# wq2012/SpectralCluster

Hardware: AMD Instinct MI355X
Metric: predict() calls/sec, n=8192 d=256 ICASSP2018 (GraphCut, eigengap k in [2,20], cosine k-means) (higher is better)
Workload: dtype f64; 1 GPU; icassp2018_graphcut_n8192_d256_k8_max20; n_samples=8192, n_features=256, parallelism=replicas x1, collectives=none

## Files before the change

### include/spectralcluster_amd.h

```cpp
#ifndef SPECTRALCLUSTER_AMD_H_
#define SPECTRALCLUSTER_AMD_H_

#include <stddef.h>
#include <stdint.h>

#ifdef __cplusplus
extern "C" {
#endif

#define SC_ABI_VERSION 10
#define SC_MAX_OPS 16
#define SC_MAX_BLUR_RADIUS 32
#define SC_MAX_EIG 128
#define SC_MAX_STAGES 16

typedef struct sc_handle_s* sc_handle;

typedef enum sc_status {
  SC_OK = 0,
  SC_ERR_INVALID = -1,
  SC_ERR_OOM = -2,
  SC_ERR_HIP = -3,
  SC_ERR_NOT_CONVERGED = -4,
  SC_ERR_UNSUPPORTED = -5,
// ... 368 lines not shown
  SC_FRONT_INFO_FREE_FORMS_S = 9,
  SC_FRONT_INFO_CROP_SOURCE = 10,
  SC_FRONT_INFO_CUT_KERNEL = 11,
  SC_FRONT_INFO_WRITTEN = 12,
  SC_FRONT_INFO_LAUNCHES = 13,
  SC_FRONT_INFO_COUNT = 16
};
typedef struct sc_front_out {
  double* a0;
  double* cropval;
  double* cut;
  double* a;
  double* s;
  double* rowmax;
  double* rowsum;
  double* c;
  double* p;
  double* t;
  int32_t info[SC_FRONT_INFO_COUNT];
} sc_front_out;
int sc_stage_front(sc_handle h, int route, const sc_config* cfg, int count, const int32_t* ns,
                   int d, const double* const* xs, const double* affinity,
                   const double* p_values, sc_front_out* outs);
enum { SC_TD_BACKTRANSFORM_GLOBAL = 1 };
int sc_stage_tridiag(sc_handle h, const double* m, int n, const double* c, const double* p,
                     double* d, double* e, double* tau, double* reflectors);
int sc_stage_tridiag_values(sc_handle h, const double* d, const double* e, int n,
                            double* values_desc);
int sc_stage_td_backtransform(sc_handle h, const double* reflectors, const double* tau, int n,
                              double* z, int cols, int flags);
int sc_stage_laplacian(sc_handle h, int laplacian_type, const double* in, int n,
                       double* out);
int sc_stage_sym_eig(sc_handle h, const double* m, int n, int count, int descend,
                     double* values, double* vectors, sc_diag* diag);
int sc_stage_eig(sc_handle h, const double* m, int n, int count, int descend,
                 double* values, double* vectors, sc_diag* diag);
int sc_random_state_doubles(uint32_t seed, int count, double* out);
int sc_uniform_choice(int n, double u);
int sc_host_symmetric_eig(const double* a, int m, double* values, double* vectors);
int sc_host_symmetric_eig_partial(const double* a, int m, int need, double* values,
                                  double* vectors);
int sc_host_tridiag_eigvectors(const double* d, const double* e, int n, const double* lam,
                               int k, double* vectors);
int sc_host_general_eig(const double* a, int m, int nvec, double* values_re, double* values_im,
                        double* vectors_re, double* vectors_im);
int sc_host_general_eig_fast(const double* a, int m, int nvec, double* values_re,
// ... 68 lines not shown
```

### spectralcluster_amd/_lib.py

```python

from __future__ import annotations

import ctypes
import os
import threading
import typing

import numpy as np

SC_MAX_OPS = 16
SC_MAX_BLUR_RADIUS = 32
SC_MAX_EIG = 128
SC_MAX_STAGES = 16

SC_OK = 0
SC_ERR_INVALID = -1
SC_ERR_OOM = -2
SC_ERR_HIP = -3
SC_ERR_NOT_CONVERGED = -4
SC_ERR_UNSUPPORTED = -5
SC_ERR_NON_FINITE = -6

STAGE_NAMES = ("affinity", "refine", "diffuse", "scaling", "eig", "kmeans",
               "total", "blur", "threshold_sym", "matvec", "affinity_gemm",
# ... 186 lines not shown
    "sc_last_error": (ctypes.c_char_p, [_handle_t]),
    "sc_synchronize": (ctypes.c_int, [_handle_t]),
    "sc_set_profiling": (ctypes.c_int, [_handle_t, ctypes.c_int]),
    "sc_set_diffuse_mode": (ctypes.c_int, [_handle_t, ctypes.c_int]),
    "sc_set_free_prune": (ctypes.c_int, [_handle_t, ctypes.c_int]),
    "sc_stage_diffuse_rowstats": (ctypes.c_int, [_handle_t, _c_double_p, ctypes.c_int,
                                                 ctypes.c_int, _c_double_p, _c_double_p,
                                                 ctypes.POINTER(ctypes.c_int32)]),
    "sc_stage_block_operator": (ctypes.c_int, [_handle_t, ctypes.c_int,
                                               ctypes.POINTER(ctypes.c_int32),
                                               ctypes.POINTER(_c_double_p),
                                               ctypes.POINTER(_c_double_p),
                                               ctypes.POINTER(_c_double_p),
                                               ctypes.POINTER(_c_double_p),
                                               ctypes.POINTER(_c_double_p),
                                               ctypes.POINTER(_c_double_p), ctypes.c_int]),
    "sc_stage_krylov_state": (ctypes.c_int, [_handle_t, ctypes.POINTER(ctypes.c_int32),
                                             _c_double_p, _c_double_p, _c_double_p, _c_double_p,
                                             _c_double_p]),
    "sc_stage_front": (ctypes.c_int, [_handle_t, ctypes.c_int, ctypes.POINTER(ScConfig),
                                      ctypes.c_int, ctypes.POINTER(ctypes.c_int32), ctypes.c_int,
                                      ctypes.POINTER(_c_double_p), _c_double_p, _c_double_p,
                                      ctypes.POINTER(ScFrontOut)]),
    "sc_stage_tridiag": (ctypes.c_int, [_handle_t, _c_double_p, ctypes.c_int, _c_double_p,
                                        _c_double_p, _c_double_p, _c_double_p, _c_double_p,
                                        _c_double_p]),
    "sc_stage_tridiag_values": (ctypes.c_int, [_handle_t, _c_double_p, _c_double_p, ctypes.c_int,
                                               _c_double_p]),
    "sc_stage_td_backtransform": (ctypes.c_int, [_handle_t, _c_double_p, _c_double_p,
                                                 ctypes.c_int, _c_double_p, ctypes.c_int,
                                                 ctypes.c_int]),
    "sc_config_default": (ctypes.c_int, [ctypes.POINTER(ScConfig)]),
    "sc_gaussian_weights": (ctypes.c_int, [ctypes.c_double,
                                           ctypes.POINTER(ctypes.c_int32),
                                           _c_double_p]),
    "sc_predict": (ctypes.c_int, [_handle_t, _c_double_p, ctypes.c_int, ctypes.c_int,
                                  ctypes.POINTER(ScConfig), _c_int64_p,
                                  ctypes.POINTER(ScDiag)]),
    "sc_set_embeddings": (ctypes.c_int, [_handle_t, _c_double_p, ctypes.c_int,
                                         ctypes.c_int]),
    "sc_predict_array": (ctypes.c_int, [_handle_t, ctypes.POINTER(ScArray),
                                        ctypes.POINTER(ScConfig), _c_int64_p,
                                        ctypes.POINTER(ScDiag)]),
    "sc_set_embeddings_array": (ctypes.c_int, [_handle_t, ctypes.POINTER(ScArray)]),
    "sc_predict_batch_arrays": (ctypes.c_int, [_handle_t, ctypes.POINTER(ScArray), ctypes.c_int,
                                               ctypes.POINTER(ScConfig),
# ... 496 lines not shown
```

### spectralcluster_amd/csrc/api.hip

```cpp
#include <algorithm>
#include <array>
#include <cmath>
#include <cstdio>
#include <cstdlib>
#include <cstring>
#include <vector>

#include <condition_variable>
#include <mutex>
#include <string>
#include <thread>

#include "handle.h"
#include "host_pool.h"

int ensure_matrices(sc_handle h, int n, int d, bool affinity_copy) {
  h->krylov_m = 0;
  const size_t ldn = matrix_ld(n);
  const size_t nn = (size_t)n * ldn * sizeof(double);
  if (affinity_copy) SC_TRY(grow(h, h->A0, nn));
  SC_TRY(grow(h, h->B1, nn));
  SC_TRY(grow(h, h->B2, nn));
  if (d > 0) {
    const size_t ldx = round_up(d, 16);
// ... 591 lines not shown
  hipStream_t s = h->stream;
  const double* cur = ptr<double>(h->A0);
  double* bufs[2] = {ptr<double>(h->B1), ptr<double>(h->B2)};
  int which = 0;
  bool symmetric = h->affinity_symmetric;
  const bool constrain_after = constraint_active(h, cfg, false);
  bool folded_rownorm = false;
  int e_begin, e_after_refine;
  const bool fine = h->profile_level >= 2;
  int eb0 = -1, eb1 = -1, et0 = -1, et1 = -1;
  h->n_mv_ev = 0;
  bool free_path = false;
  const double* amax_of = nullptr;
  const double* digits_of = nullptr;
  float diffuse_ms_events[SC_MAX_OPS][2];
  int n_diffuse = 0;
  ev_rec(h, &e_begin);
  const bool blur_fast = (cfg->blur_radius == 4 || cfg->blur_radius == 8) && n >= 128;
  const double* pending_diag = nullptr;
  bool have_partials = false;
  bool have_row_stats = false;
  int crop_source = 0, cut_kernel = 0;
  h->last_blur = BlurLaunch();
  if (resume) {
    cur = resume->matrix;
    symmetric = resume->symmetric;
    folded_rownorm = resume->folded_rownorm;
    which = resume->scratch == bufs[0] ? 0 : 1;
    if (resume->free_op) h->free_checked = false;
  }
  for (int i = 0; i < (resume ? 0 : cfg->n_ops); ++i) {
    const int op = cfg->ops[i];
    const int next = i + 1 < cfg->n_ops ? cfg->ops[i + 1] : 0;
    const int next2 = i + 2 < cfg->n_ops ? cfg->ops[i + 2] : 0;
    const bool thr_sym_fusable = true;
    const bool partials_usable = cfg->threshold_type == SC_THRESHOLD_ROW_MAX &&
                                 !cfg->preserve_diagonal;
    if (op == SC_OP_ROW_WISE_NORMALIZE && symmetric && i == cfg->n_ops - 1 &&
        !constrain_after) {
      folded_rownorm = true;
      continue;
    }
    if (op == SC_OP_CROP_DIAGONAL && next == SC_OP_GAUSSIAN_BLUR && blur_fast) {
      if (cur == ptr<double>(h->A0) && h->have_cropval) {
        pending_diag = ptr<double>(h->cropval);
        crop_source = 1;
      } else {
        launch_crop_value(s, cur, n, ld, ptr<double>(h->dvec));
        pending_diag = ptr<double>(h->dvec);
        crop_source = 2;
      }
      have_partials = false;
      continue;
    }
    double* out = bufs[which];
    which ^= 1;
    int e0 = -1, e1 = -1;
    bool keep_cur = false;
    if (op == SC_OP_DIFFUSE) ev_rec(h, &e0);
    if (op == SC_OP_GAUSSIAN_BLUR && blur_fast) {
      const bool want = next == SC_OP_ROW_WISE_THRESHOLD && next2 == SC_OP_SYMMETRIZE &&
                        partials_usable;
      SC_TRY(upload_blur_weights(h, cfg));
      if (fine) ev_rec(h, &eb0);
      have_partials = launch_gaussian_blur_fused(s, cur, out, n, ld, cfg->blur_radius,
                                                 ptr<double>(h->blurw), pending_diag,
                                                 want ? ptr<double>(h->rmpart) : nullptr,
                                                 &h->last_blur);
      if (fine) ev_rec(h, &eb1);
      pending_diag = nullptr;
      SC_TRY(check_last(h, "blur launch"));
    } else if (op == SC_OP_ROW_WISE_THRESHOLD && next == SC_OP_SYMMETRIZE && thr_sym_fusable) {
      if (cfg->threshold_type == SC_THRESHOLD_PERCENTILE)
        launch_cut_percentile(s, cur, n, ld, cfg->p_percentile, ptr<double>(h->cut),
                              cfg->preserve_diagonal);
      else if (have_partials && partials_usable)
        launch_cut_from_partials(s, ptr<double>(h->rmpart), n,
                                 blur_tile_columns(n, cfg->blur_radius),
                                 cfg->p_percentile, ptr<double>(h->cut));
      else
        launch_cut_from_rows(s, cur, n, ld, cfg->p_percentile, ptr<double>(h->cut),
                             cfg->preserve_diagonal);
      cut_kernel = cfg->threshold_type == SC_THRESHOLD_PERCENTILE
                       ? 3 : (have_partials && partials_usable ? 1 : 2);
      const bool amax_known =
          cfg->threshold_type == SC_THRESHOLD_ROW_MAX && h->affinity_from_embeddings &&
          !h->constraint_applied && cfg->p_percentile > 0.0 && cfg->soft_multiplier >= 0.0 &&
          cfg->soft_multiplier <= 1.0 && i + 2 < cfg->n_ops && cfg->ops[i + 2] == SC_OP_DIFFUSE &&
          free_diffuse_wanted(h, cfg, n, make_eig_request(cfg));
      const bool fuse_digits =
          amax_known && !constrain_after && !front_only &&
          (i + 2 == cfg->n_ops - 1 ||
           (i + 2 == cfg->n_ops - 2 && cfg->ops[i + 3] == SC_OP_ROW_WISE_NORMALIZE));
      const double amax_floor = (cfg->binarize || cfg->preserve_diagonal) ? 1.0 : 0.0;
      if (fuse_digits)
        SC_TRY(free_fused_prepare(h, s, n, ptr<double>(h->cut), cfg->p_percentile, amax_floor));
      if (fine) ev_rec(h, &et0);
      if (fuse_digits)
        launch_threshold_symmetrize_digits(s, cur, out, n, ld, ptr<double>(h->cut),
                                           cfg->soft_multiplier, cfg->binarize,
                                           cfg->symmetrize_type, cfg->preserve_diagonal,
                                           ptr<signed char>(h->fq), ptr<double>(h->fscal),
                                           ptr<double>(h->fypart), ptr<int>(h->frpart),
                                           ptr<double>(h->fq2part), ptr<double>(h->fmx64));
      else
        launch_threshold_symmetrize(s, cur, out, n, ld, ptr<double>(h->cut),
                                    cfg->soft_multiplier, cfg->binarize, cfg->symmetrize_type,
                                    cfg->preserve_diagonal);
      if (fine) ev_rec(h, &et1);
      SC_TRY(check_last(h, "threshold+symmetrize launch"));
      if (fuse_digits) {
        amax_of = out;
        digits_of = out;
      } else if (amax_known) {
        SC_TRY(ensure_free(h, n));
        launch_free_amax_from_cut(s, ptr<double>(h->cut), n, cfg->p_percentile, amax_floor,
                                  ptr<double>(h->fscal));
        amax_of = out;
      }
      have_partials = false;
      cur = out;
// ... 641 lines not shown
```

### spectralcluster_amd/csrc/blur.hip

```cpp
#include <algorithm>
#include <cstring>

#include "dpp.h"
#include "sc_internal.h"

namespace sc {

constexpr int TH = 32;
constexpr int TW = 64;


__global__ __launch_bounds__(256) void k_gaussian_blur(
    const double* __restrict__ in, double* __restrict__ out, int n, int ld,
    int radius, const double* __restrict__ weights) {
  extern __shared__ __attribute__((aligned(16))) double smem[];
  const int R = radius;
  const int HW = TW + 2 * R;
  const int HH = TH + 2 * R;
  double* tile = smem;
  double* mid = smem + HH * HW;
  double* w = mid + TH * HW;

  const int i0 = blockIdx.y * TH;
  const int j0 = blockIdx.x * TW;
// ... 130 lines not shown
#pragma unroll
      for (int e = 0; e < 4; ++e) dst[e] = row[gjin[e]];
    }
    if (diag != nullptr) {
#pragma unroll
      for (int e = 0; e < 4; ++e)
        if (gjin[e] == gi) dst[e] = diag[gi];
    }
  };
  double win[S][4];
#pragma unroll
  for (int q = 0; q < S - 1; ++q) load_row(r0 - R + q, win[q]);
  const int gjo0 = j0 + q0 - R;
  const bool lane_ok = q0 >= R && q0 + 3 < 256 - R;
  const bool full_store = lane_ok && gjo0 + 3 < n;
  for (int o = r0; o < rend; o += S) {
#pragma unroll
    for (int u = 0; u < S; ++u) {
      const int gi = o + u;
      if (gi >= rend) break;
      load_row(gi + R + kAhead, win[(u + S - 1) % S]);
      double t[4];
#pragma unroll
      for (int e = 0; e < 4; ++e) {
        double acc = win[(u + R) % S][e] * w[0];
#pragma unroll
        for (int j = R; j >= 1; --j)
          acc += (win[(u + R - j) % S][e] + win[(u + R + j) % S][e]) * w[j];
        t[e] = acc;
      }
      double ext[(2 * NB + 1) * 4];
#pragma unroll
      for (int e = 0; e < 4; ++e) ext[NB * 4 + e] = t[e];
#pragma unroll
      for (int e = 0; e < 4; ++e) {
        double below = t[e], above = t[e];
#pragma unroll
        for (int d = 1; d <= NB; ++d) {
          below = lane_from_below(below);
          above = lane_from_above(above);
          ext[(NB - d) * 4 + e] = below;
          ext[(NB + d) * 4 + e] = above;
        }
      }
      double res[4];
      double m = -INFINITY;
#pragma unroll
      for (int e = 0; e < 4; ++e) {
        double acc = ext[NB * 4 + e] * w[0];
#pragma unroll
        for (int j = R; j >= 1; --j)
          acc += (ext[NB * 4 + e - j] + ext[NB * 4 + e + j]) * w[j];
        res[e] = acc;
        if (lane_ok && gjo0 + e < n) m = fmax(m, acc);
      }
      double* orow = out + (size_t)gi * ld + gjo0;
      if (out == nullptr) {
      } else if (full_store) {
        *reinterpret_cast<double2*>(orow) = make_double2(res[0], res[1]);
        *reinterpret_cast<double2*>(orow + 2) = make_double2(res[2], res[3]);
      } else if (lane_ok) {
#pragma unroll
        for (int e = 0; e < 4; ++e)
          if (gjo0 + e < n) orow[e] = res[e];
      }
      if (rowmax != nullptr) {
        m = wave_max_to_last(m);
        if (lane == 63) rowmax[(size_t)gi * ncols + bx] = m;
      }
    }
  }
}
template <int R>
__global__ __launch_bounds__(256) void k_gaussian_blur_stream(
    const double* __restrict__ in, double* __restrict__ out, int n, int ld,
// ... 37 lines not shown
  if (j >= n) return;
  auto at = [&](int e) { return AXIS == 0 ? in[(size_t)e * ld + j] : in[(size_t)i * ld + e]; };
  out[(size_t)i * ld + j] = blur_line_point(at, AXIS == 0 ? i : j, n, radius, weights);
}

void launch_gaussian_blur_any_radius(hipStream_t s, const double* in, double* tmp, double* out,
                                     int n, int ld, int radius, const double* weights_dev) {
  dim3 grid((n + 255) / 256, n);
  hipLaunchKernelGGL(k_gaussian_blur_axis<0>, grid, dim3(256), 0, s, in, tmp, n, ld, radius,
                     weights_dev);
  hipLaunchKernelGGL(k_gaussian_blur_axis<1>, grid, dim3(256), 0, s, tmp, out, n, ld, radius,
                     weights_dev);
}

void launch_gaussian_blur(hipStream_t s, const double* in, double* out, int n,
                          int ld, int radius, const double* weights_dev) {
  launch_gaussian_blur_fused(s, in, out, n, ld, radius, weights_dev, nullptr, nullptr);
}

int blur_tile_columns(int n, int radius) {
  const int ow = (n >= kStreamMinN ? 256 : 64) - 2 * radius;
  return (n + ow - 1) / ow;
}

bool launch_gaussian_blur_fused(hipStream_t s, const double* in, double* out, int n, int ld,
                                int radius, const double* weights_dev, const double* diag,
                                double* rowmax_partials, BlurLaunch* taken) {
  dim3 grid((n + TW - 1) / TW, (n + TH - 1) / TH);
  if (taken) *taken = BlurLaunch{0, 0};
  if ((radius == 4 || radius == 8) && n >= kStreamMinN) {
    const int strips = blur_tile_columns(n, radius);
    int rows = stream_rows_per_wave((long long)strips * n, radius);
    const int per_round = 256 * (radius == 4 ? 3 : 2);
    while (rows < kStreamRowsMax) {
      const long long wgs = (long long)strips * ((n + 4 * rows - 1) / (4 * rows));
      if (wgs <= per_round || wgs % per_round == 0 || wgs % per_round > per_round * 3 / 4) break;
      ++rows;
    }
    dim3 sgrid(strips, (n + 4 * rows - 1) / (4 * rows));
    if (taken) *taken = BlurLaunch{2, rows};
    if (radius == 4)
      hipLaunchKernelGGL((k_gaussian_blur_stream<4>), sgrid, dim3(256), 0, s, in, out, n, ld,
                         weights_dev, diag, rowmax_partials, rows);
    else
      hipLaunchKernelGGL((k_gaussian_blur_stream<8>), sgrid, dim3(256), 0, s, in, out, n, ld,
                         weights_dev, diag, rowmax_partials, rows);
// ... 63 lines not shown
```

### spectralcluster_amd/csrc/handle.h

```cpp
#ifndef SPECTRALCLUSTER_AMD_HANDLE_H_
#define SPECTRALCLUSTER_AMD_HANDLE_H_

#include <algorithm>
#include <array>
#include <cmath>
#include <cstdio>
#include <cstdlib>
#include <cstring>
#include <string>
#include <vector>

#include "sc_internal.h"

using namespace sc;

struct DevBuf {
  void* p = nullptr;
  size_t bytes = 0;
};

constexpr int kKgenBufs = 12;
constexpr int kGroupBanks = 2;
constexpr int kGroupLanes = 3;

// ... 93 lines not shown
  int gconv_hist[16] = {0};
  int gconv_seen = 0;
  hipEvent_t ev[48];
  int nev = 0;
  StageEvents stage_events;
  int profile_level = 1;
  int mv_ev[16][2];
  int n_mv_ev = 0;
  int aff_ev[2] = {-1, -1};
  int blurw_radius = -1;
  double blurw_host[2 * SC_MAX_BLUR_RADIUS + 1];
  int krnd_k = -1, krnd_trials = -1;
  int kfirst_n = -1, kfirst = 0;
  int diffuse_mode = -1;
  DevBuf fq, ft32, fy1, fR, fscal, fwords, fcand, fY, fsplit, fypart, frpart;
  int free_prune = -1;
  DevBuf fq2part, fmx64, ftau64, fplan;
  int* h_free = nullptr;
  bool free_checked = false;
  int free_ev[5] = {-1, -1, -1, -1, -1};
  int krylov_m = 0, krylov_n = 0, krylov_cycles = 0, krylov_ahead = 0;
  bool krylov_free = false;
  BlurLaunch last_blur;
};

inline void ev_rec(sc_handle h, int* slot) {
  if (h->nev < 48) {
    hipEventRecord(h->ev[h->nev], h->stream);
    *slot = h->nev++;
  } else {
    *slot = -1;
  }
}
inline float ev_ms(sc_handle h, int a, int b) {
  if (a < 0 || b < 0) return 0.f;
  float ms = 0.f;
  hipEventElapsedTime(&ms, h->ev[a], h->ev[b]);
  return ms;
}

constexpr int kTilemapTableMax = 64;
constexpr int kMaxCols = 128;
inline int matrix_ld(int n) {
  int ld = round_up(n, 16);
  if (ld % 512 == 0) ld += 16;
  return ld;
// ... 245 lines not shown
```

### spectralcluster_amd/csrc/rowops.hip

```cpp
#include <algorithm>
#include <cstring>

#include "dpp.h"
#include "sc_internal.h"

namespace sc {

constexpr int kRowThreads = 256;

__device__ __forceinline__ double wave_max(double v) {
#pragma unroll
  for (int o = 32; o > 0; o >>= 1) v = fmax(v, __shfl_xor(v, o));
  return v;
}
__device__ __forceinline__ double wave_sum(double v) {
#pragma unroll
  for (int o = 32; o > 0; o >>= 1) v += __shfl_xor(v, o);
  return v;
}
__device__ __forceinline__ double block_max(double v, double* sm) {
  v = wave_max(v);
  __syncthreads();
  if ((threadIdx.x & 63) == 0) sm[threadIdx.x >> 6] = v;
  __syncthreads();
// ... 313 lines not shown
    hb[w] = (signed char)h;
    lb[w] = (signed char)l;
  }
  signed char* dst = dg.Q + (size_t)row * dg.pitch + (size_t)blk * 128 + c0;
  *reinterpret_cast<short*>(dst) = (short)((unsigned char)hb[0] | ((unsigned short)(unsigned char)hb[1] << 8));
  *reinterpret_cast<short*>(dst + 64) = (short)((unsigned char)lb[0] | ((unsigned short)(unsigned char)lb[1] << 8));
  const double ys = half_sum_to_last(v0 + v1);
  const int rs = half_sum_to_last(qv[0] + qv[1]);
  const double q2s = half_sum_to_last(q2);
  if (lane0) {
    dg.ypart[(size_t)blk * (kTsTile * dg.nblk) + row] = ys;
    dg.rpart[(size_t)blk * (kTsTile * dg.nblk) + row] = rs;
    dg.q2part[(size_t)blk * (kTsTile * dg.nblk) + row] = q2s;
  }
  return q2s;
}
__device__ __forceinline__ void ts_store_mx(const TsDigits& dg, const double* sm, int group,
                                            int blk) {
  double m = sm[0];
#pragma unroll
  for (int u = 1; u < 8; ++u) m = fmax(m, sm[u]);
  dg.mx64[(size_t)group * dg.nblk + blk] = sqrt(m) * (1.0 + 0x1p-52);
}
template <bool DIGITS>
__device__ __forceinline__ void threshold_symmetrize_body(
    const double* __restrict__ in, double* __restrict__ out, int n, int ld,
    const double* __restrict__ cut, double mult, int binarize, int symtype, int ntiles,
    int preserve_diag, const TsDigits dg) {
  __shared__ double tT[kTsTile][kTsTile + 1];
  __shared__ double smax[2][8];
  double q2m = 0.0;
  const bool digits = DIGITS && dg.Q != nullptr;
  const int id = blockIdx.x;
  const double b2 = 2.0 * ntiles + 1.0;
  int ti = (int)((b2 - sqrt(b2 * b2 - 8.0 * id)) * 0.5);
  ti = ti < 0 ? 0 : (ti >= ntiles ? ntiles - 1 : ti);
  auto off = [&](int t) { return t * ntiles - (t * (t - 1)) / 2; };
  while (ti > 0 && off(ti) > id) --ti;
  while (ti + 1 < ntiles && off(ti + 1) <= id) ++ti;
  const int tj = ti + (id - off(ti));
  const int bi = ti * kTsTile, bj = tj * kTsTile;
  const int tx = threadIdx.x & 31, ty = threadIdx.x >> 5;
  const int c0 = 2 * tx;
  const bool diag_tile = ti == tj;
  double2 a[8], b[8];
  double ca[8], cb[8];
#pragma unroll
  for (int q = 0; q < 8; ++q) {
    const int r = ty + 8 * q;
    const int gi = bi + r, gj = bj + c0;
    a[q] = (gi < n && gj < n) ? *reinterpret_cast<const double2*>(in + (size_t)gi * ld + gj)
                              : make_double2(0.0, 0.0);
    ca[q] = gi < n ? cut[gi] : 0.0;
  }
  if (!diag_tile) {
#pragma unroll
    for (int q = 0; q < 8; ++q) {
      const int r = ty + 8 * q;
      const int gi = bj + r, gj = bi + c0;
      b[q] = (gi < n && gj < n) ? *reinterpret_cast<const double2*>(in + (size_t)gi * ld + gj)
                                : make_double2(0.0, 0.0);
      cb[q] = gi < n ? cut[gi] : 0.0;
    }
  }
  auto thr = [&](double v, double c, int gi, int gj) {
    if (!(gi < n && gj < n)) return 0.0;
    v = v < c ? v * mult : (binarize ? 1.0 : v);
    if (preserve_diag && gi == gj) v = 1.0;
    return v;
  };
#pragma unroll
  for (int q = 0; q < 8; ++q) {
    const int r = ty + 8 * q;
    a[q].x = thr(a[q].x, ca[q], bi + r, bj + c0);
    a[q].y = thr(a[q].y, ca[q], bi + r, bj + c0 + 1);
    if (diag_tile) {
      b[q] = a[q];
    } else {
      b[q].x = thr(b[q].x, cb[q], bj + r, bi + c0);
      b[q].y = thr(b[q].y, cb[q], bj + r, bi + c0 + 1);
    }
    tT[r][c0] = b[q].x;
    tT[r][c0 + 1] = b[q].y;
  }
  __syncthreads();
  double sigma = 0.0;
  if (digits) {
// ... 27 lines not shown
#pragma unroll
  for (int q = 0; q < 8; ++q) {
    const int r = ty + 8 * q;
    tT[r][c0] = a[q].x;
    tT[r][c0 + 1] = a[q].y;
  }
  __syncthreads();
#pragma unroll
  for (int q = 0; q < 8; ++q) {
    const int r = ty + 8 * q;
    const int gi = bj + r, gj = bi + c0;
    const double2 o = make_double2(tT[c0][r], tT[c0 + 1][r]);
    if (gi < n && gj + 1 < n)
      *reinterpret_cast<double2*>(out + (size_t)gi * ld + gj) = o;
    else if (gi < n && gj < n)
      out[(size_t)gi * ld + gj] = o.x;
    if (digits) q2m = fmax(q2m, ts_digits(dg, sigma, gi, ti, c0, o.x, o.y, tx == 31));
  }
  if (digits) {
    if (tx == 31) smax[1][ty] = q2m;
    __syncthreads();
    if (threadIdx.x == 0) ts_store_mx(dg, smax[1], tj, ti);
  }
}
__global__ __launch_bounds__(256) void k_threshold_symmetrize(
    const double* __restrict__ in, double* __restrict__ out, int n, int ld,
    const double* __restrict__ cut, double mult, int binarize, int symtype, int ntiles,
    int preserve_diag) {
  threshold_symmetrize_body<false>(in, out, n, ld, cut, mult, binarize, symtype, ntiles,
                                   preserve_diag, TsDigits{});
}
__global__ __launch_bounds__(256) void k_threshold_symmetrize_digits(
    const double* __restrict__ in, double* __restrict__ out, int n, int ld,
    const double* __restrict__ cut, double mult, int binarize, int symtype, int ntiles,
    int preserve_diag, const TsDigits dg) {
  threshold_symmetrize_body<true>(in, out, n, ld, cut, mult, binarize, symtype, ntiles,
                                  preserve_diag, dg);
}
__device__ __forceinline__ void free_partials_reduce_body(
    const double* __restrict__ ypart, const int* __restrict__ rpart, int n, int nblk,
    double* __restrict__ y1, double* __restrict__ R, unsigned long long* __restrict__ rmax_bits,
    const FreeSegs segs) {
  __shared__ double sy[4][64];
  __shared__ double sq[4][64];
  __shared__ long long sr[4][64];
  const int r = threadIdx.x & 63, qd = threadIdx.x >> 6;
// ... 573 lines not shown
                     cut, mult, binarize, preserve_diag);
}
void launch_threshold_symmetrize(hipStream_t s, const double* in, double* out, int n, int ld,
                                 const double* cut, double mult, int binarize, int symtype,
                                 int preserve_diag) {
  const int t = (n + kTsTile - 1) / kTsTile;
  hipLaunchKernelGGL(k_threshold_symmetrize, dim3(t * (t + 1) / 2), dim3(256), 0, s, in, out,
                     n, ld, cut, mult, binarize, symtype, t, preserve_diag);
}
void launch_threshold_symmetrize_digits(hipStream_t s, const double* in, double* out, int n, int ld,
                                        const double* cut, double mult, int binarize, int symtype,
                                        int preserve_diag, signed char* Q, double* scal,
                                        double* ypart, int* rpart, double* q2part,
                                        double* mx64) {
  const int t = (n + kTsTile - 1) / kTsTile;
  const size_t pitch = (size_t)2 * t * kTsTile;
  const int rows_padded = (n + 127) / 128 * 128;
  if (rows_padded > t * kTsTile)
    hipMemsetAsync(Q + (size_t)t * kTsTile * pitch, 0, (size_t)(rows_padded - t * kTsTile) * pitch, s);
  const TsDigits dg{Q, pitch, t, scal, ypart, rpart, q2part, mx64};
  hipLaunchKernelGGL(k_threshold_symmetrize_digits, dim3(t * (t + 1) / 2), dim3(256), 0, s, in,
                     out, n, ld, cut, mult, binarize, symtype, t, preserve_diag, dg);
}
void launch_free_partials_reduce(hipStream_t s, const double* ypart, const int* rpart, int n,
                                 double* y1, double* R, double* scal, const FreeSegs& segs) {
  const int nblk = (n + kTsTile - 1) / kTsTile;
  hipLaunchKernelGGL(k_free_partials_reduce, dim3(nblk), dim3(256), 0, s, ypart, rpart, n,
                     nblk, y1, R, reinterpret_cast<unsigned long long*>(scal) + 2, segs);
}
void launch_row_normalize(hipStream_t s, const double* in, double* out, int n,
                          int ld) {
  hipLaunchKernelGGL(k_row_normalize, dim3(n), dim3(kRowThreads), 0, s, in, out, n,
                     ld);
}
void launch_row_stats(hipStream_t s, const double* in, int n, int ld,
                      double* rowmax, double* rowsum) {
  hipLaunchKernelGGL(k_row_stats, dim3(n), dim3(kRowThreads), 0, s, in, n, ld,
                     rowmax, rowsum);
}
void launch_scaling_vectors(hipStream_t s, const double* rowmax,
                            const double* rowsum, int n, int laplacian_type,
                            int row_normalized, double* c, double* p, double* t, int* flags,
                            int* symflag) {
  hipLaunchKernelGGL(k_scaling_vectors, dim3((n + 255) / 256), dim3(256), 0, s,
                     rowmax, rowsum, n, laplacian_type, row_normalized, c, p, t, flags, symflag);
}
// ... 125 lines not shown
```

### spectralcluster_amd/csrc/sc_internal.h

```cpp
#pragma once

#include <hip/hip_runtime.h>

#include "switches.h"
#include <stdint.h>

#include <mutex>
#include <string>
#include <vector>

#include "../../include/spectralcluster_amd.h"

namespace sc {

constexpr int kWave = 64;
constexpr int kEigBlock = 8;
constexpr int kEigBasisCap = 128;
constexpr int kLdq = kEigBasisCap + kEigBlock;
constexpr int kDenseMax = 128;
constexpr int kHostRR = 64;
constexpr int kHostRRSingle = kEigBasisCap;
constexpr int kGenMax = 64;
constexpr int kMaxVectors = 64;
constexpr int kProjBlocks = 128;
// ... 71 lines not shown

void launch_normalize_rows(hipStream_t s, const double* X, int ldx, int n, int d,
                           double* Xn, int* bad_rows = nullptr);
void launch_crop_diagonal(hipStream_t s, const double* in, double* out, int n,
                          int ld);
void launch_gaussian_blur(hipStream_t s, const double* in, double* out, int n,
                          int ld, int radius, const double* weights_dev);
struct BlurLaunch {
  int kernel = -1, rows = 0;
};
__device__ __forceinline__ int reflect_index(int j, int n) {
  const int period = 2 * n;
  j %= period;
  if (j < 0) j += period;
  return j < n ? j : period - 1 - j;
}
template <class At>
__device__ __forceinline__ double blur_line_point(At at, int e, int n, int radius,
                                                  const double* __restrict__ weights) {
  double t = at(e) * weights[radius];
  for (int q = radius; q >= 1; --q)
    t += (at(reflect_index(e - q, n)) + at(reflect_index(e + q, n))) * weights[radius - q];
  return t;
}
bool launch_gaussian_blur_fused(hipStream_t s, const double* in, double* out, int n, int ld,
                                int radius, const double* weights_dev, const double* diag,
                                double* rowmax_partials, BlurLaunch* taken = nullptr);
int blur_tile_columns(int n, int radius);
void launch_gaussian_blur_any_radius(hipStream_t s, const double* in, double* tmp, double* out,
                                     int n, int ld, int radius, const double* weights_dev);
void launch_crop_value(hipStream_t s, const double* in, int n, int ld, double* dvec);
void launch_cut_from_partials(hipStream_t s, const double* partials, int n, int ntiles,
                              double p, double* cut);
void launch_cut_from_rows(hipStream_t s, const double* in, int n, int ld, double p,
                          double* cut, int zero_diag);
void launch_cut_percentile(hipStream_t s, const double* in, int n, int ld, double p,
                           double* cut, int zero_diag);
void launch_row_threshold_cut(hipStream_t s, const double* in, double* out, int n, int ld,
                              const double* cut, double mult, int binarize,
                              int preserve_diag);
void launch_threshold_symmetrize(hipStream_t s, const double* in, double* out, int n, int ld,
                                 const double* cut, double mult, int binarize, int symtype,
                                 int preserve_diag);
void launch_threshold_symmetrize_digits(hipStream_t s, const double* in, double* out, int n, int ld,
                                        const double* cut, double mult, int binarize, int symtype,
                                        int preserve_diag, signed char* Q, double* scal,
                                        double* ypart, int* rpart, double* q2part,
                                        double* mx64);
struct FreeSegs;
void launch_free_partials_reduce(hipStream_t s, const double* ypart, const int* rpart, int n,
                                 double* y1, double* R, double* scal, const FreeSegs& segs);
void launch_row_threshold(hipStream_t s, const double* in, double* out, int n,
                          int ld, double p, double mult, int binarize,
                          int preserve_diag);
void launch_symmetrize(hipStream_t s, const double* in, double* out, int n, int ld,
                       int type);

void launch_affinity_integration(hipStream_t s, const double* a, const double* q, double* out,
                                 int n, int ld, int type);
void launch_affinity_integration_band(hipStream_t s, const double* a, const double* band,
                                      double* out, int n, int ld, int type);
void launch_cp_band_product(hipStream_t s, const double* tt, const double* band, double* x,
                            int n, int ld);
void launch_cp_prepare(hipStream_t s, const double* a, const double* deg, double alpha,
                       double* p, double* t0, int n, int ld);
void launch_cp_adjust(hipStream_t s, const double* tqt, const double* a, double scale,
                      double* out, int n, int ld);
void launch_transpose(hipStream_t s, const double* in, double* out, int n, int ld);
void launch_symmetry_flag(hipStream_t s, const double* in, int n, int ld, int* flag);
void launch_row_normalize(hipStream_t s, const double* in, double* out, int n,
                          int ld);
// ... 584 lines not shown
```

### spectralcluster_amd/csrc/stage_front.hip

```cpp
#include "batch_internal.h"

namespace {
struct FrontWhere {
  sc_handle h = nullptr;
  int n = 0, ld = 0;
  const double* a0 = nullptr;
  const double* cropval = nullptr;
  const double* cut = nullptr;
  const double* a = nullptr;
  const double* s = nullptr;
  int diffuse_path = SC_DIFFUSE_PATH_NONE;
  bool symmetric = true, folded_rownorm = false, free_op = false, digits_fused = false;
  BlurLaunch blur;
  int crop_source = 0, cut_kernel = 0;
};
FrontWhere front_where(sc_handle lead, sc_handle hz, int n, const FrontResult& fr) {
  FrontWhere w;
  w.h = hz;
  w.n = n;
  w.ld = hz->ldn;
  w.a0 = ptr<double>(hz->A0);
  w.cropval = ptr<double>(hz->cropval);
  w.cut = fr.cut_kernel != 0 ? ptr<double>(hz->cut) : nullptr;
  w.a = ptr<double>(hz->B2);
// ... 87 lines not shown
                        const double* const* xs, sc_front_out* outs) {
  const EigRequest rq = make_eig_request(cfg);
  std::vector<int> ns(ns32, ns32 + count), idx(count);
  int largest = 0, smallest = ns[0];
  for (int z = 0; z < count; ++z) {
    idx[z] = z;
    largest = std::max(largest, ns[z]);
    smallest = std::min(smallest, ns[z]);
    if (!sym_group_eligible(ns[z], rq))
      return fail(h, SC_ERR_UNSUPPORTED, "sc_stage_front: a member outside the grouped route");
  }
  if (constraint_active(h, cfg, true) || constraint_active(h, cfg, false) ||
      !grouped_front_covers(cfg) || !blur_group_front_supported(smallest, cfg->blur_radius))
    return fail(h, SC_ERR_UNSUPPORTED,
                "sc_stage_front: the grouped front covers the ICASSP2018 sequence (blur radius 4 "
                "or 8, RowMax) on members of n >= 256");
  h->sweep_slot.clear();
  const std::vector<sc_array> arrays = host_f64_arrays(xs, ns.data(), d, count);
  SC_TRY(ensure_bank_stream(h, 0));
  SC_TRY(reserve_bank_arenas(h, cfg, rq, 0, count, largest, d, nullptr));
  SC_TRY(upload_group_blur_weights(h, cfg));
  Member mb[kGroupMax];
  h->last_blur = BlurLaunch();
  const int rc = enqueue_front_grouped(h, arrays.data(), ns.data(), d, cfg, nullptr, idx.data(),
                                       count, 0, mb, 0);
  SC_HIP(h, hipStreamSynchronize(h->gbank_stream[0]));
  SC_TRY(rc);
  for (int z = 0; z < count; ++z)
    SC_TRY(front_copy_out(h, front_where(h, mb[z].h, ns[z], mb[z].front), outs + z));
  return SC_OK;
}

int stage_front_sweep(sc_handle h, const sc_config* cfg, int count, int n, int d, const double* x,
                      const double* p_values, sc_front_out* outs) {
  SC_TRY(sc_set_embeddings(h, x, n, d));
  SC_TRY(sc_compute_affinity(h));
  const EigRequest rq = make_eig_request(cfg);
  const SweepPlan plan = sweep_plan(h, cfg, count, rq);
  if (!plan.grouped)
    return fail(h, SC_ERR_UNSUPPORTED,
                "sc_stage_front: sc_eig_ncluster_sweep would evaluate this level one by one");
  h->last_blur = BlurLaunch();
  const double* crop = nullptr;
  int crop_source = 0;
  if (plan.icassp) SC_TRY(sweep_shared_blur(h, cfg, &crop, &crop_source));
  FrontItem fi[kGroupMax];
  GemmGroupItem dif[kGroupMax];
  GroupEigMember em[kGroupMax];
  FrontResult taken[kGroupMax];
  memset(fi, 0, sizeof(fi));
  bool out_of_memory = false;
  SC_TRY(sweep_round_members(h, cfg, plan, rq, p_values, count, fi, dif, em, &out_of_memory));
  if (out_of_memory)
    return fail(h, SC_ERR_OOM, "sc_stage_front: the round's member arenas do not fit");
  SC_TRY(sweep_round_front(h, cfg, plan, p_values, count, fi, dif, em, taken));
  SC_HIP(h, hipStreamSynchronize(h->stream));
  for (int z = 0; z < count; ++z) {
    FrontResult fr = taken[z];
    fr.symmetric = true;
    fr.folded_rownorm = plan.icassp;
    fr.free_op = em[z].free_op;
    fr.crop_source = crop_source;
    FrontWhere w = front_where(h, em[z].h, n, fr);
    w.a0 = ptr<double>(h->A0);
    w.cropval = crop;
    SC_TRY(front_copy_out(h, w, outs + z));
  }
  return SC_OK;
}

int stage_front_short_sweep(sc_handle h, const sc_config* cfg, int count, int n, int d,
                            const double* x, const double* p_values, sc_front_out* outs) {
  SC_TRY(sc_set_embeddings(h, x, n, d));
  SC_TRY(sc_compute_affinity(h));
  const EigRequest rq = make_eig_request(cfg);
  const SweepPlan plan = sweep_plan(h, cfg, count, rq);
  if (!plan.short_level)
    return fail(h, SC_ERR_UNSUPPORTED,
                "sc_stage_front: sc_eig_ncluster_sweep would not run this level as short pairs");
  h->sweep_slot.clear();
  h->last_blur = BlurLaunch();
  ShortShared sh;
  SC_TRY(sweep_short_shared(h, cfg, plan, &sh));
  std::vector<FrontItem> fi(kShortWidth);
  std::vector<GemmGroupItem> dif(kShortWidth);
  std::vector<GroupEigMember> em(kShortWidth);
  memset(fi.data(), 0, fi.size() * sizeof(FrontItem));
  bool out_of_memory = false;
  SC_TRY(sweep_short_front(h, cfg, plan, rq, sh, p_values, count, fi.data(), dif.data(),
                           em.data(), &out_of_memory));
  if (out_of_memory)
    return fail(h, SC_ERR_OOM, "sc_stage_front: the level's member arenas do not fit");
  SC_HIP(h, hipStreamSynchronize(h->stream));
  for (int z = 0; z < count; ++z) {
    FrontResult fr;
    fr.symmetric = true;
    fr.folded_rownorm = fr.diffuse_explicit = plan.icassp;
    fr.crop_source = sh.crop_source;
    fr.cut_kernel = 4;
    FrontWhere w = front_where(h, em[z].h, n, fr);
    w.a0 = ptr<double>(h->A0);
    w.cropval = sh.crop;
    SC_TRY(front_copy_out(h, w, outs + z));
  }
// ... 64 lines not shown
    if (ns[z] <= 0 || (xs && !xs[z]))
      return fail(h, SC_ERR_INVALID, "sc_stage_front: every member needs rows");
  if (xs ? d <= 0 : (route != SC_FRONT_ROUTE_SINGLE || !affinity))
    return fail(h, SC_ERR_INVALID,
                "sc_stage_front: embeddings (n, d), or an affinity on the single route");
  switch (route) {
    case SC_FRONT_ROUTE_SINGLE:
      if (count != 1) return fail(h, SC_ERR_INVALID, "sc_stage_front: the single route takes one");
      return stage_front_single(h, cfg, ns[0], d, xs ? xs[0] : nullptr, affinity, outs);
    case SC_FRONT_ROUTE_GROUPED:
      return stage_front_grouped(h, cfg, count, ns, d, xs, outs);
    case SC_FRONT_ROUTE_SWEEP:
      if (!p_values) return fail(h, SC_ERR_INVALID, "sc_stage_front: p_values is NULL");
      return stage_front_sweep(h, cfg, count, ns[0], d, xs[0], p_values, outs);
    case SC_FRONT_ROUTE_SHORT_SWEEP:
      if (!p_values) return fail(h, SC_ERR_INVALID, "sc_stage_front: p_values is NULL");
      return stage_front_short_sweep(h, cfg, count, ns[0], d, xs[0], p_values, outs);
    case SC_FRONT_ROUTE_SHORT_WAVE:
      if (!xs) return fail(h, SC_ERR_INVALID, "sc_stage_front: the short wave takes embeddings");
      return stage_front_short_wave(h, cfg, count, ns, d, xs, outs);
  }
  return fail(h, SC_ERR_INVALID, "sc_stage_front: unknown route");
}
```

### spectralcluster_amd/csrc/switches.h

```cpp
#ifndef SPECTRALCLUSTER_AMD_SWITCHES_H_
#define SPECTRALCLUSTER_AMD_SWITCHES_H_

#include <cstdlib>
#include <cstring>

namespace sc {
namespace sw {

inline int eig_trace() {
  static const int v = getenv("SC_EIG_TRACE") ? std::max(1, atoi(getenv("SC_EIG_TRACE"))) : 0;
  return v;
}
inline bool kmeans_trace() {
  static const bool v = getenv("SC_KMEANS_TRACE") != nullptr;
  return v;
}
inline bool group_trace() {
  static const bool v = getenv("SC_GROUP_TRACE") != nullptr;
  return v;
}
inline bool eig_host_chain() {
  static const bool v = getenv("SC_EIG_HOST_CHAIN") != nullptr;
  return v;
}
// ... 29 lines not shown
  return v;
}
inline int diffuse_free_min_n_group() {
  static const int v =
      getenv("SC_DIFFUSE_FREE_MIN_N") ? atoi(getenv("SC_DIFFUSE_FREE_MIN_N")) : 1536;
  return v;
}
inline int gen_dense_max_n() {
  static const int v = getenv("SC_GEN_DENSE_MAX_N") ? atoi(getenv("SC_GEN_DENSE_MAX_N")) : 512;
  return v;
}
inline bool free_no_prune() {
  static const bool v = getenv("SC_FREE_NO_PRUNE") != nullptr;
  return v;
}
inline bool sweep_one_by_one() {
  static const bool v = getenv("SC_SWEEP_ONE_BY_ONE") != nullptr;
  return v;
}
inline bool short_front_memberwise() {
  static const bool v = getenv("SC_SHORT_FRONT_MEMBERWISE") != nullptr;
  return v;
}

}
}

#endif
```

Before: 393.7 calls/s.

## Fuse Gaussian blur into the threshold-symmetrize kernel to skip writing the blurred matrix

Adds a kernel that loads a haloed tile of the cropped affinity into LDS, applies the radius-4 separable Gaussian blur in place, then runs the existing threshold/symmetrize/digits tail on the blurred tiles. When conditions hold, the standalone blur kernel still computes row-max partials but no longer writes the blurred n×n matrix, and the threshold kernel reads the raw affinity instead. This removes one full dense f64 write and one read of an 8192×8192 matrix. The cost is redundant halo loads and recomputation of the blur for both the tile and its transposed partner, plus more LDS use per block.

Result: faster. 400.4 calls/s (median of 6 runs) (+1.7%).

```diff
diff --git a/include/spectralcluster_amd.h b/include/spectralcluster_amd.h
--- a/include/spectralcluster_amd.h
+++ b/include/spectralcluster_amd.h
@@ -414,6 +414,7 @@
 int sc_stage_front(sc_handle h, int route, const sc_config* cfg, int count, const int32_t* ns,
                    int d, const double* const* xs, const double* affinity,
                    const double* p_values, sc_front_out* outs);
+int sc_last_front_route(sc_handle h);
 enum { SC_TD_BACKTRANSFORM_GLOBAL = 1 };
 int sc_stage_tridiag(sc_handle h, const double* m, int n, const double* c, const double* p,
                      double* d, double* e, double* tau, double* reflectors);
diff --git a/spectralcluster_amd/_lib.py b/spectralcluster_amd/_lib.py
--- a/spectralcluster_amd/_lib.py
+++ b/spectralcluster_amd/_lib.py
@@ -232,6 +232,7 @@
                                       ctypes.c_int, ctypes.POINTER(ctypes.c_int32), ctypes.c_int,
                                       ctypes.POINTER(_c_double_p), _c_double_p, _c_double_p,
                                       ctypes.POINTER(ScFrontOut)]),
+    "sc_last_front_route": (ctypes.c_int, [_handle_t]),
     "sc_stage_tridiag": (ctypes.c_int, [_handle_t, _c_double_p, ctypes.c_int, _c_double_p,
                                         _c_double_p, _c_double_p, _c_double_p, _c_double_p,
                                         _c_double_p]),
diff --git a/spectralcluster_amd/csrc/api.hip b/spectralcluster_amd/csrc/api.hip
--- a/spectralcluster_amd/csrc/api.hip
+++ b/spectralcluster_amd/csrc/api.hip
@@ -637,6 +637,8 @@
   bool have_row_stats = false;
   int crop_source = 0, cut_kernel = 0;
   h->last_blur = BlurLaunch();
+  h->last_front_fused = false;
+  const double* blur_in_threshold = nullptr;
   if (resume) {
     cur = resume->matrix;
     symmetric = resume->symmetric;
@@ -677,8 +679,18 @@
       const bool want = next == SC_OP_ROW_WISE_THRESHOLD && next2 == SC_OP_SYMMETRIZE &&
                         partials_usable;
       SC_TRY(upload_blur_weights(h, cfg));
+      const bool fused = want && !front_only && !sw::front_write_blur() &&
+                         blur_front_fusable(n, cfg->blur_radius) && cur == ptr<double>(h->A0) &&
+                         crop_source == 1 && pending_diag == ptr<double>(h->cropval) &&
+                         h->affinity_from_embeddings && h->affinity_symmetric &&
+                         !h->constraint_applied;
+      if (fused) {
+        blur_in_threshold = pending_diag;
+        keep_cur = true;
+      }
       if (fine) ev_rec(h, &eb0);
-      have_partials = launch_gaussian_blur_fused(s, cur, out, n, ld, cfg->blur_radius,
+      have_partials = launch_gaussian_blur_fused(s, cur, fused ? nullptr : out, n, ld,
+                                                 cfg->blur_radius,
                                                  ptr<double>(h->blurw), pending_diag,
                                                  want ? ptr<double>(h->rmpart) : nullptr,
                                                  &h->last_blur);
@@ -711,7 +723,16 @@
       if (fuse_digits)
         SC_TRY(free_fused_prepare(h, s, n, ptr<double>(h->cut), cfg->p_percentile, amax_floor));
       if (fine) ev_rec(h, &et0);
-      if (fuse_digits)
+      if (blur_in_threshold != nullptr) {
+        launch_blur_threshold_symmetrize(
+            s, cur, blur_in_threshold, ptr<double>(h->blurw), out, n, ld, ptr<double>(h->cut),
+            cfg->soft_multiplier, cfg->binarize, cfg->symmetrize_type,
+            fuse_digits ? ptr<signed char>(h->fq) : nullptr, ptr<double>(h->fscal),
+            ptr<double>(h->fypart), ptr<int>(h->frpart), ptr<double>(h->fq2part),
+            ptr<double>(h->fmx64));
+        h->last_front_fused = true;
+        blur_in_threshold = nullptr;
+      } else if (fuse_digits)
         launch_threshold_symmetrize_digits(s, cur, out, n, ld, ptr<double>(h->cut),
                                            cfg->soft_multiplier, cfg->binarize,
                                            cfg->symmetrize_type, cfg->preserve_diagonal,
diff --git a/spectralcluster_amd/csrc/blur.hip b/spectralcluster_amd/csrc/blur.hip
--- a/spectralcluster_amd/csrc/blur.hip
+++ b/spectralcluster_amd/csrc/blur.hip
@@ -176,13 +176,8 @@
       load_row(gi + R + kAhead, win[(u + S - 1) % S]);
       double t[4];
 #pragma unroll
-      for (int e = 0; e < 4; ++e) {
-        double acc = win[(u + R) % S][e] * w[0];
-#pragma unroll
-        for (int j = R; j >= 1; --j)
-          acc += (win[(u + R - j) % S][e] + win[(u + R + j) % S][e]) * w[j];
-        t[e] = acc;
-      }
+      for (int e = 0; e < 4; ++e)
+        t[e] = blur_taps<R>([&](int k) { return win[(u + R + k) % S][e]; }, w);
       double ext[(2 * NB + 1) * 4];
 #pragma unroll
       for (int e = 0; e < 4; ++e) ext[NB * 4 + e] = t[e];
@@ -201,10 +196,7 @@
       double m = -INFINITY;
 #pragma unroll
       for (int e = 0; e < 4; ++e) {
-        double acc = ext[NB * 4 + e] * w[0];
-#pragma unroll
-        for (int j = R; j >= 1; --j)
-          acc += (ext[NB * 4 + e - j] + ext[NB * 4 + e + j]) * w[j];
+        const double acc = blur_taps<R>([&](int k) { return ext[NB * 4 + e + k]; }, w);
         res[e] = acc;
         if (lane_ok && gjo0 + e < n) m = fmax(m, acc);
       }
@@ -288,6 +280,8 @@
   const int ow = (n >= kStreamMinN ? 256 : 64) - 2 * radius;
   return (n + ow - 1) / ow;
 }
+
+bool blur_front_fusable(int n, int radius) { return radius == 4 && n >= kStreamMinN; }
 
 bool launch_gaussian_blur_fused(hipStream_t s, const double* in, double* out, int n, int ld,
                                 int radius, const double* weights_dev, const double* diag,
diff --git a/spectralcluster_amd/csrc/handle.h b/spectralcluster_amd/csrc/handle.h
--- a/spectralcluster_amd/csrc/handle.h
+++ b/spectralcluster_amd/csrc/handle.h
@@ -139,6 +139,7 @@
   int krylov_m = 0, krylov_n = 0, krylov_cycles = 0, krylov_ahead = 0;
   bool krylov_free = false;
   BlurLaunch last_blur;
+  bool last_front_fused = false;
 };
 
 inline void ev_rec(sc_handle h, int* slot) {
diff --git a/spectralcluster_amd/csrc/rowops.hip b/spectralcluster_amd/csrc/rowops.hip
--- a/spectralcluster_amd/csrc/rowops.hip
+++ b/spectralcluster_amd/csrc/rowops.hip
@@ -359,47 +359,28 @@
   for (int u = 1; u < 8; ++u) m = fmax(m, sm[u]);
   dg.mx64[(size_t)group * dg.nblk + blk] = sqrt(m) * (1.0 + 0x1p-52);
 }
-template <bool DIGITS>
-__device__ __forceinline__ void threshold_symmetrize_body(
-    const double* __restrict__ in, double* __restrict__ out, int n, int ld,
-    const double* __restrict__ cut, double mult, int binarize, int symtype, int ntiles,
-    int preserve_diag, const TsDigits dg) {
-  __shared__ double tT[kTsTile][kTsTile + 1];
-  __shared__ double smax[2][8];
-  double q2m = 0.0;
-  const bool digits = DIGITS && dg.Q != nullptr;
-  const int id = blockIdx.x;
+__device__ __forceinline__ void ts_tile_pair(int id, int ntiles, int* pti, int* ptj) {
   const double b2 = 2.0 * ntiles + 1.0;
   int ti = (int)((b2 - sqrt(b2 * b2 - 8.0 * id)) * 0.5);
   ti = ti < 0 ? 0 : (ti >= ntiles ? ntiles - 1 : ti);
   auto off = [&](int t) { return t * ntiles - (t * (t - 1)) / 2; };
   while (ti > 0 && off(ti) > id) --ti;
   while (ti + 1 < ntiles && off(ti + 1) <= id) ++ti;
-  const int tj = ti + (id - off(ti));
+  *pti = ti;
+  *ptj = ti + (id - off(ti));
+}
+template <bool DIGITS>
+__device__ __forceinline__ void threshold_symmetrize_tail(
+    double2 (&a)[8], double2 (&b)[8], const double (&ca)[8], const double (&cb)[8],
+    double (*tT)[kTsTile + 1], double (*smax)[8], double* __restrict__ out, int n, int ld,
+    double mult, int binarize, int symtype, int ti, int tj, int preserve_diag,
+    const TsDigits& dg) {
+  double q2m = 0.0;
+  const bool digits = DIGITS && dg.Q != nullptr;
   const int bi = ti * kTsTile, bj = tj * kTsTile;
   const int tx = threadIdx.x & 31, ty = threadIdx.x >> 5;
   const int c0 = 2 * tx;
   const bool diag_tile = ti == tj;
-  double2 a[8], b[8];
-  double ca[8], cb[8];
-#pragma unroll
-  for (int q = 0; q < 8; ++q) {
-    const int r = ty + 8 * q;
-    const int gi = bi + r, gj = bj + c0;
-    a[q] = (gi < n && gj < n) ? *reinterpret_cast<const double2*>(in + (size_t)gi * ld + gj)
-                              : make_double2(0.0, 0.0);
-    ca[q] = gi < n ? cut[gi] : 0.0;
-  }
-  if (!diag_tile) {
-#pragma unroll
-    for (int q = 0; q < 8; ++q) {
-      const int r = ty + 8 * q;
-      const int gi = bj + r, gj = bi + c0;
-      b[q] = (gi < n && gj < n) ? *reinterpret_cast<const double2*>(in + (size_t)gi * ld + gj)
-                                : make_double2(0.0, 0.0);
-      cb[q] = gi < n ? cut[gi] : 0.0;
-    }
-  }
   auto thr = [&](double v, double c, int gi, int gj) {
     if (!(gi < n && gj < n)) return 0.0;
     v = v < c ? v * mult : (binarize ? 1.0 : v);
@@ -473,6 +454,163 @@
     __syncthreads();
     if (threadIdx.x == 0) ts_store_mx(dg, smax[1], tj, ti);
   }
+}
+template <bool DIGITS>
+__device__ __forceinline__ void threshold_symmetrize_body(
+    const double* __restrict__ in, double* __restrict__ out, int n, int ld,
+    const double* __restrict__ cut, double mult, int binarize, int symtype, int ntiles,
+    int preserve_diag, const TsDigits dg) {
+  __shared__ double tT[kTsTile][kTsTile + 1];
+  __shared__ double smax[2][8];
+  int ti, tj;
+  ts_tile_pair(blockIdx.x, ntiles, &ti, &tj);
+  const int bi = ti * kTsTile, bj = tj * kTsTile;
+  const int tx = threadIdx.x & 31, ty = threadIdx.x >> 5;
+  const int c0 = 2 * tx;
+  const bool diag_tile = ti == tj;
+  double2 a[8], b[8];
+  double ca[8], cb[8];
+#pragma unroll
+  for (int q = 0; q < 8; ++q) {
+    const int r = ty + 8 * q;
+    const int gi = bi + r, gj = bj + c0;
+    a[q] = (gi < n && gj < n) ? *reinterpret_cast<const double2*>(in + (size_t)gi * ld + gj)
+                              : make_double2(0.0, 0.0);
+    ca[q] = gi < n ? cut[gi] : 0.0;
+  }
+  if (!diag_tile) {
+#pragma unroll
+    for (int q = 0; q < 8; ++q) {
+      const int r = ty + 8 * q;
+      const int gi = bj + r, gj = bi + c0;
+      b[q] = (gi < n && gj < n) ? *reinterpret_cast<const double2*>(in + (size_t)gi * ld + gj)
+                                : make_double2(0.0, 0.0);
+      cb[q] = gi < n ? cut[gi] : 0.0;
+    }
+  }
+  threshold_symmetrize_tail<DIGITS>(a, b, ca, cb, tT, smax, out, n, ld, mult, binarize, symtype,
+                                    ti, tj, preserve_diag, dg);
+}
+
+constexpr int kBtR = 4;
+constexpr int kBtHalo = kTsTile + 2 * kBtR;
+constexpr int kBtLdT = kBtHalo + 1;
+constexpr int kBtLdM = kBtHalo + 2;
+constexpr int kBtStrip = 16;
+constexpr size_t kBtLdsBytes =
+    sizeof(double) * ((size_t)kBtHalo * kBtLdT + (size_t)kBtStrip * kBtLdM + 2 * 8);
+static_assert(kBtHalo * kBtLdT >= kTsTile * (kTsTile + 1), "the tail's tile reuses T");
+static_assert(kBtStrip == 16 && 2 * kBtHalo <= 256, "two 8-row segments, one thread per line each");
+template <bool TRANSPOSED>
+__device__ __forceinline__ void bt_blur_side(const double* T, double* M,
+                                             const double (&w)[kBtR + 1], double2 (&dst)[8]) {
+  const int tid = threadIdx.x;
+  constexpr int step = TRANSPOSED ? 1 : kBtLdT;
+  constexpr int line = TRANSPOSED ? kBtLdT : 1;
+  const int c0 = 2 * (tid & 31), ty = tid >> 5;
+  const int seg = tid / kBtHalo, h = tid - seg * kBtHalo;
+#pragma unroll
+  for (int s = 0; s < kTsTile / kBtStrip; ++s) {
+    if (tid < 2 * kBtHalo) {
+      const double* src = T + h * line + (kBtStrip * s + 8 * seg) * step;
+      double x[8 + 2 * kBtR];
+#pragma unroll
+      for (int k = 0; k < 8 + 2 * kBtR; ++k) x[k] = src[k * step];
+#pragma unroll
+      for (int m = 0; m < 8; ++m)
+        M[(8 * seg + m) * kBtLdM + h] = blur_taps<kBtR>([&](int k) { return x[m + kBtR + k]; }, w);
+    }
+    __syncthreads();
+    __builtin_amdgcn_sched_barrier(0);
+#pragma unroll
+    for (int qq = 0; qq < 2; ++qq) {
+      const double* row = M + (ty + 8 * qq) * kBtLdM + c0;
+      double x[2 * kBtR + 2];
+#pragma unroll
+      for (int k = 0; k < kBtR + 1; ++k) {
+        const double2 p = *reinterpret_cast<const double2*>(row + 2 * k);
+        x[2 * k] = p.x;
+        x[2 * k + 1] = p.y;
+      }
+      dst[2 * s + qq] = make_double2(blur_taps<kBtR>([&](int k) { return x[kBtR + k]; }, w),
+                                     blur_taps<kBtR>([&](int k) { return x[kBtR + 1 + k]; }, w));
+      asm volatile("" : "+v"(dst[2 * s + qq].x), "+v"(dst[2 * s + qq].y));
+    }
+    __syncthreads();
+    __builtin_amdgcn_sched_barrier(0);
+  }
+}
+template <bool DIGITS>
+__global__ __launch_bounds__(256, 3) void k_blur_threshold_symmetrize(
+    const double* __restrict__ a0, const double* __restrict__ cropval,
+    const double* __restrict__ weights, double* __restrict__ out, int n, int ld,
+    const double* __restrict__ cut, double mult, int binarize, int symtype, int ntiles,
+    const TsDigits dg) {
+  extern __shared__ __attribute__((aligned(16))) double bt_smem[];
+  double* T = bt_smem;
+  double* M = T + kBtHalo * kBtLdT;
+  double(*smax)[8] = reinterpret_cast<double(*)[8]>(M + kBtStrip * kBtLdM);
+  double(*tT)[kTsTile + 1] = reinterpret_cast<double(*)[kTsTile + 1]>(T);
+  int ti, tj;
+  ts_tile_pair(blockIdx.x, ntiles, &ti, &tj);
+  const int bi = ti * kTsTile, bj = tj * kTsTile;
+  const int tid = threadIdx.x;
+  const int ty = tid >> 5;
+  const bool diag_tile = ti == tj;
+  double w[kBtR + 1];
+#pragma unroll
+  for (int j = 0; j <= kBtR; ++j) w[j] = weights[kBtR - j];
+  double ca[8], cb[8];
+#pragma unroll
+  for (int q = 0; q < 8; ++q) {
+    const int gi = bi + ty + 8 * q, gk = bj + ty + 8 * q;
+    ca[q] = gi < n ? cut[gi] : 0.0;
+    cb[q] = (!diag_tile && gk < n) ? cut[gk] : 0.0;
+  }
+  auto reflect = [&](int g) {
+    g = g < 0 ? -g - 1 : g;
+    g = g >= n ? 2 * n - 1 - g : g;
+    return g < 0 ? 0 : (g >= n ? n - 1 : g);
+  };
+  const bool interior = bi >= kBtR && bi + kTsTile + kBtR <= n && bj + kTsTile + kBtR <= n;
+  if (interior) {
+    constexpr int kPairs = kBtHalo / 2, kTotal = kBtHalo * kPairs;
+    constexpr int kPer = (kTotal + 255) / 256;
+    double2 v[kPer];
+#pragma unroll
+    for (int k = 0; k < kPer; ++k) {
+      const int e = tid + 256 * k;
+      if (e < kTotal) {
+        const int h = e / kPairs, p = e - h * kPairs;
+        v[k] = *reinterpret_cast<const double2*>(a0 + (size_t)(bi - kBtR + h) * ld +
+                                                 (bj - kBtR + 2 * p));
+      }
+    }
+#pragma unroll
+    for (int k = 0; k < kPer; ++k) {
+      const int e = tid + 256 * k;
+      if (e < kTotal) {
+        const int h = e / kPairs, p = e - h * kPairs;
+        const int gi = bi - kBtR + h, gj = bj - kBtR + 2 * p;
+        if (gi == gj) v[k].x = cropval[gi];
+        if (gi == gj + 1) v[k].y = cropval[gi];
+        T[h * kBtLdT + 2 * p] = v[k].x;
+        T[h * kBtLdT + 2 * p + 1] = v[k].y;
+      }
+    }
+  } else {
+    for (int e = tid; e < kBtHalo * kBtHalo; e += 256) {
+      const int h = e / kBtHalo, c = e - h * kBtHalo;
+      const int gi = reflect(bi - kBtR + h), gj = reflect(bj - kBtR + c);
+      T[h * kBtLdT + c] = gi == gj ? cropval[gi] : a0[(size_t)gi * ld + gj];
+    }
+  }
+  __syncthreads();
+  double2 a[8], b[8];
+  bt_blur_side<false>(T, M, w, a);
+  if (!diag_tile) bt_blur_side<true>(T, M, w, b);
+  threshold_symmetrize_tail<DIGITS>(a, b, ca, cb, tT, smax, out, n, ld, mult, binarize, symtype,
+                                    ti, tj, 0, dg);
 }
 __global__ __launch_bounds__(256) void k_threshold_symmetrize(
     const double* __restrict__ in, double* __restrict__ out, int n, int ld,
@@ -1092,6 +1230,29 @@
   hipLaunchKernelGGL(k_threshold_symmetrize_digits, dim3(t * (t + 1) / 2), dim3(256), 0, s, in,
                      out, n, ld, cut, mult, binarize, symtype, t, preserve_diag, dg);
 }
+void launch_blur_threshold_symmetrize(hipStream_t s, const double* a0, const double* cropval,
+                                      const double* weights_dev, double* out, int n, int ld,
+                                      const double* cut, double mult, int binarize, int symtype,
+                                      signed char* Q, double* scal, double* ypart, int* rpart,
+                                      double* q2part, double* mx64) {
+  const int t = (n + kTsTile - 1) / kTsTile;
+  const size_t pitch = (size_t)2 * t * kTsTile;
+  const dim3 grid(t * (t + 1) / 2);
+  if (Q == nullptr) {
+    SC_OPT_IN_LDS(k_blur_threshold_symmetrize<false>, kBtLdsBytes);
+    hipLaunchKernelGGL(k_blur_threshold_symmetrize<false>, grid, dim3(256), kBtLdsBytes, s, a0,
+                       cropval, weights_dev, out, n, ld, cut, mult, binarize, symtype, t,
+                       TsDigits{});
+    return;
+  }
+  const int rows_padded = (n + 127) / 128 * 128;
+  if (rows_padded > t * kTsTile)
+    hipMemsetAsync(Q + (size_t)t * kTsTile * pitch, 0, (size_t)(rows_padded - t * kTsTile) * pitch, s);
+  const TsDigits dg{Q, pitch, t, scal, ypart, rpart, q2part, mx64};
+  SC_OPT_IN_LDS(k_blur_threshold_symmetrize<true>, kBtLdsBytes);
+  hipLaunchKernelGGL(k_blur_threshold_symmetrize<true>, grid, dim3(256), kBtLdsBytes, s, a0,
+                     cropval, weights_dev, out, n, ld, cut, mult, binarize, symtype, t, dg);
+}
 void launch_free_partials_reduce(hipStream_t s, const double* ypart, const int* rpart, int n,
                                  double* y1, double* R, double* scal, const FreeSegs& segs) {
   const int nblk = (n + kTsTile - 1) / kTsTile;
diff --git a/spectralcluster_amd/csrc/sc_internal.h b/spectralcluster_amd/csrc/sc_internal.h
--- a/spectralcluster_amd/csrc/sc_internal.h
+++ b/spectralcluster_amd/csrc/sc_internal.h
@@ -117,6 +117,13 @@
   for (int q = radius; q >= 1; --q)
     t += (at(reflect_index(e - q, n)) + at(reflect_index(e + q, n))) * weights[radius - q];
   return t;
+}
+template <int R, class At>
+__device__ __forceinline__ double blur_taps(At at, const double (&w)[R + 1]) {
+  double acc = at(0) * w[0];
+#pragma unroll
+  for (int j = R; j >= 1; --j) acc += (at(-j) + at(j)) * w[j];
+  return acc;
 }
 bool launch_gaussian_blur_fused(hipStream_t s, const double* in, double* out, int n, int ld,
                                 int radius, const double* weights_dev, const double* diag,
@@ -142,6 +149,12 @@
                                         int preserve_diag, signed char* Q, double* scal,
                                         double* ypart, int* rpart, double* q2part,
                                         double* mx64);
+bool blur_front_fusable(int n, int radius);
+void launch_blur_threshold_symmetrize(hipStream_t s, const double* a0, const double* cropval,
+                                      const double* weights_dev, double* out, int n, int ld,
+                                      const double* cut, double mult, int binarize, int symtype,
+                                      signed char* Q, double* scal, double* ypart, int* rpart,
+                                      double* q2part, double* mx64);
 struct FreeSegs;
 void launch_free_partials_reduce(hipStream_t s, const double* ypart, const int* rpart, int n,
                                  double* y1, double* R, double* scal, const FreeSegs& segs);
diff --git a/spectralcluster_amd/csrc/stage_front.hip b/spectralcluster_amd/csrc/stage_front.hip
--- a/spectralcluster_amd/csrc/stage_front.hip
+++ b/spectralcluster_amd/csrc/stage_front.hip
@@ -133,6 +133,7 @@
   SC_TRY(upload_group_blur_weights(h, cfg));
   Member mb[kGroupMax];
   h->last_blur = BlurLaunch();
+  h->last_front_fused = false;
   const int rc = enqueue_front_grouped(h, arrays.data(), ns.data(), d, cfg, nullptr, idx.data(),
                                        count, 0, mb, 0);
   SC_HIP(h, hipStreamSynchronize(h->gbank_stream[0]));
@@ -152,6 +153,7 @@
     return fail(h, SC_ERR_UNSUPPORTED,
                 "sc_stage_front: sc_eig_ncluster_sweep would evaluate this level one by one");
   h->last_blur = BlurLaunch();
+  h->last_front_fused = false;
   const double* crop = nullptr;
   int crop_source = 0;
   if (plan.icassp) SC_TRY(sweep_shared_blur(h, cfg, &crop, &crop_source));
@@ -191,6 +193,7 @@
                 "sc_stage_front: sc_eig_ncluster_sweep would not run this level as short pairs");
   h->sweep_slot.clear();
   h->last_blur = BlurLaunch();
+  h->last_front_fused = false;
   ShortShared sh;
   SC_TRY(sweep_short_shared(h, cfg, plan, &sh));
   std::vector<FrontItem> fi(kShortWidth);
@@ -301,3 +304,5 @@
   }
   return fail(h, SC_ERR_INVALID, "sc_stage_front: unknown route");
 }
+
+extern "C" int sc_last_front_route(sc_handle h) { return h && h->last_front_fused ? 1 : 0; }
diff --git a/spectralcluster_amd/csrc/switches.h b/spectralcluster_amd/csrc/switches.h
--- a/spectralcluster_amd/csrc/switches.h
+++ b/spectralcluster_amd/csrc/switches.h
@@ -75,6 +75,10 @@
   static const bool v = getenv("SC_SHORT_FRONT_MEMBERWISE") != nullptr;
   return v;
 }
+inline bool front_write_blur() {
+  static const bool v = getenv("SC_FRONT_WRITE_BLUR") != nullptr;
+  return v;
+}
 
 }
 }
```
